# OFA-Sys/ONE-PEACE

Hardware: NVIDIA H100
Metric: encoder_samples_per_sec (higher is better)
Workload: dtype bf16

## Files before the change

one_peace_b200/csrc/common.cuh:

```cuda
#pragma once
#include <cuda.h>
#include <cuda_bf16.h>
#include <cuda_runtime.h>
#include <stdint.h>
#include <stdio.h>
#include <stdlib.h>

#define OPB_DEVICE __device__ __forceinline__

#define OPB_OK 0
#define OPB_ERR_INVALID 1
#define OPB_ERR_CUDA 2
#define OPB_ERR_UNSUPPORTED 3

namespace opb {

OPB_DEVICE uint32_t smem_u32(const void* p) {
  return static_cast<uint32_t>(__cvta_generic_to_shared(p));
}
OPB_DEVICE uint32_t lane_id() { return threadIdx.x & 31; }

OPB_DEVICE bool elect_one() {
  uint32_t pred = 0;
  asm volatile(
      "{\n\t"
      ".reg .pred P;\n\t"
      "elect.sync _|P, 0xffffffff;\n\t"
      "selp.b32 %0, 1, 0, P;\n\t"
      "}\n"
      : "=r"(pred));
  return pred != 0;
}

OPB_DEVICE uint64_t globaltimer_ns() {
  uint64_t t;
  asm volatile("mov.u64 %0, %%globaltimer;" : "=l"(t));
  return t;
}

OPB_DEVICE void mbar_init(uint64_t* bar, uint32_t count) {
  asm volatile("mbarrier.init.shared::cta.b64 [%0], %1;" ::"r"(smem_u32(bar)), "r"(count) : "memory");
}
OPB_DEVICE void fence_barrier_init() { asm volatile("fence.mbarrier_init.release.cluster;" ::: "memory"); }
OPB_DEVICE void fence_proxy_async() { asm volatile("fence.proxy.async.shared::cta;" ::: "memory"); }

OPB_DEVICE void mbar_arrive_expect_tx(uint64_t* bar, uint32_t bytes) {
  asm volatile("mbarrier.arrive.expect_tx.shared::cta.b64 _, [%0], %1;" ::"r"(smem_u32(bar)), "r"(bytes)
               : "memory");
}
OPB_DEVICE void mbar_arrive(uint64_t* bar) {
  asm volatile("mbarrier.arrive.shared::cta.b64 _, [%0];" ::"r"(smem_u32(bar)) : "memory");
}
OPB_DEVICE bool mbar_try_wait(uint64_t* bar, uint32_t parity) {
  uint32_t ok;
  asm volatile(
      "{\n\t"
      ".reg .pred P;\n\t"
      "mbarrier.try_wait.parity.shared::cta.b64 P, [%1], %2;\n\t"
      "selp.b32 %0, 1, 0, P;\n\t"
      "}\n"
      : "=r"(ok)
      : "r"(smem_u32(bar)), "r"(parity)
      : "memory");
  return ok != 0;
}

#ifndef OPB_WATCHDOG_NS
#define OPB_WATCHDOG_NS 4000000000ull
#endif
OPB_DEVICE void mbar_wait(uint64_t* bar, uint32_t parity) {
  if (mbar_try_wait(bar, parity)) return;
  uint64_t t0 = globaltimer_ns();
  uint32_t spins = 0;
  while (!mbar_try_wait(bar, parity)) {
    if ((++spins & 0x3ff) == 0) {
      if (globaltimer_ns() - t0 > OPB_WATCHDOG_NS) {
        printf("[opb] mbarrier watchdog: block %d thread %d bar@%u parity %u\n", (int)blockIdx.x,
               (int)threadIdx.x, smem_u32(bar), parity);
        __trap();
      }
    }
  }
}

OPB_DEVICE void mbar_wait_quiet(uint64_t* bar, uint32_t parity) {
  if (mbar_try_wait(bar, parity)) return;
  const uint64_t t0 = globaltimer_ns();
  while (!mbar_try_wait(bar, parity)) {
    if (globaltimer_ns() - t0 > OPB_WATCHDOG_NS) __trap();
  }
}

OPB_DEVICE uint64_t wgmma_desc_sw128(uint32_t smem_addr, uint32_t lbo) {
  uint64_t d = 0;
  d |= static_cast<uint64_t>((smem_addr & 0x3FFFFu) >> 4);
  d |= static_cast<uint64_t>((lbo >> 4) & 0x3FFFu) << 16;
  d |= static_cast<uint64_t>(1024 >> 4) << 32;
  d |= static_cast<uint64_t>(1) << 62;
  return d;
}

OPB_DEVICE void wgmma_fence() { asm volatile("wgmma.fence.sync.aligned;" ::: "memory"); }
OPB_DEVICE void wgmma_commit() { asm volatile("wgmma.commit_group.sync.aligned;" ::: "memory"); }
template <int N>
OPB_DEVICE void wgmma_wait() { asm volatile("wgmma.wait_group.sync.aligned %0;" ::"n"(N) : "memory"); }

static inline int sm_count() {
  static int n = 0;
  if (n == 0) {
    int dev = 0;
    cudaGetDevice(&dev);
    cudaDeviceGetAttribute(&n, cudaDevAttrMultiProcessorCount, dev);
  }
  return n;
}

OPB_DEVICE void tma_prefetch_desc(const CUtensorMap* m) {
  asm volatile("prefetch.tensormap [%0];" ::"l"(reinterpret_cast<uint64_t>(m)) : "memory");
}

OPB_DEVICE void tma_load_2d(const CUtensorMap* m, uint64_t* bar, void* dst, int32_t c0, int32_t c1) {
  asm volatile(
      "cp.async.bulk.tensor.2d.shared::cluster.global.mbarrier::complete_tx::bytes [%0], [%1, {%3, %4}], [%2];"
      :
      : "r"(smem_u32(dst)), "l"(reinterpret_cast<uint64_t>(m)), "r"(smem_u32(bar)), "r"(c0), "r"(c1)
      : "memory");
}
OPB_DEVICE void tma_load_3d(const CUtensorMap* m, uint64_t* bar, void* dst, int32_t c0, int32_t c1, int32_t c2) {
  asm volatile(
      "cp.async.bulk.tensor.3d.shared::cluster.global.mbarrier::complete_tx::bytes [%0], [%1, {%3, %4, %5}], [%2];"
      :
      : "r"(smem_u32(dst)), "l"(reinterpret_cast<uint64_t>(m)), "r"(smem_u32(bar)), "r"(c0), "r"(c1), "r"(c2)
      : "memory");
}
// ... 63 lines not shown
```

one_peace_b200/csrc/gemm_wgmma.cu:

```cuda
#include "common.cuh"
#include "gemm.h"

#include <mutex>

namespace opb {

constexpr int kBlockM = 128;
constexpr int kBlockN = 256;
constexpr int kBlockK = 64;
constexpr int kStages = 4;
constexpr int kStagesTmaOut = 3;
constexpr int kABytes = kBlockM * kBlockK * 2;
constexpr int kBBytes = kBlockN * kBlockK * 2;
constexpr int kStageBytes = kABytes + kBBytes;
constexpr int kThreads = 384;
constexpr int kBandM = 8;
constexpr int kResidBatch = 16;

struct EpiOperands {
  float2 row[kBlockM];
  float colsum[kBlockN], bias[kBlockN], gamma[kBlockN], colscale[kBlockN];
};
constexpr int kStagerThreads = 96;
constexpr int kOutBoxBytes = 64 * 128;
constexpr int kOutStageBytes = 4 * kOutBoxBytes;
constexpr int smem_bytes(int stages, bool tma_out) {
  return stages * kStageBytes + (tma_out ? 2 * kOutStageBytes : 0) + 1024 + 2 * sizeof(EpiOperands) + 1024;
}
constexpr int kSmemBytes = smem_bytes(kStages, false);
constexpr int kSmemBytesTmaOut = smem_bytes(kStagesTmaOut, true);
static_assert(kSmemBytesTmaOut <= 227 * 1024, "output staging does not fit next to the stage ring");

struct GemmGeom {
  int M, N, K;
  int kb_inner;
  int num_k_blocks;
  int groups;
  int a_group_c0;
  int b_group_rows;
  int a_mn;
  int b_mn;
  int kb_per_piece;
  int m_pad;
  float* split_ws;
};

OPB_DEVICE void fence_acc(float (&d)[128]) {
#pragma unroll
  for (int i = 0; i < 128; ++i) asm volatile("" : "+f"(d[i])::"memory");
}

template <int TA, int TB>
OPB_DEVICE void wgmma_m64n256k16(float (&d)[128], uint64_t desc_a, uint64_t desc_b, uint32_t scale_d) {
  asm volatile(
      "{\n\t"
      ".reg .pred p;\n\t"
      "setp.ne.b32 p, %130, 0;\n\t"
      "wgmma.mma_async.sync.aligned.m64n256k16.f32.bf16.bf16 "
      "{"
      "%0, %1, %2, %3, %4, %5, %6, %7, %8, %9, %10, %11, %12, %13, %14, %15, "
      "%16, %17, %18, %19, %20, %21, %22, %23, %24, %25, %26, %27, %28, %29, %30, %31, "
      "%32, %33, %34, %35, %36, %37, %38, %39, %40, %41, %42, %43, %44, %45, %46, %47, "
      "%48, %49, %50, %51, %52, %53, %54, %55, %56, %57, %58, %59, %60, %61, %62, %63, "
      "%64, %65, %66, %67, %68, %69, %70, %71, %72, %73, %74, %75, %76, %77, %78, %79, "
      "%80, %81, %82, %83, %84, %85, %86, %87, %88, %89, %90, %91, %92, %93, %94, %95, "
      "%96, %97, %98, %99, %100, %101, %102, %103, %104, %105, %106, %107, %108, %109, %110, %111, "
      "%112, %113, %114, %115, %116, %117, %118, %119, %120, %121, %122, %123, %124, %125, %126, %127"
      "}, %128, %129, p, 1, 1, %131, %132;\n\t"
      "}\n"
      : "+f"(d[0]), "+f"(d[1]), "+f"(d[2]), "+f"(d[3]), "+f"(d[4]), "+f"(d[5]), "+f"(d[6]), "+f"(d[7]),
        "+f"(d[8]), "+f"(d[9]), "+f"(d[10]), "+f"(d[11]), "+f"(d[12]), "+f"(d[13]), "+f"(d[14]), "+f"(d[15]),
        "+f"(d[16]), "+f"(d[17]), "+f"(d[18]), "+f"(d[19]), "+f"(d[20]), "+f"(d[21]), "+f"(d[22]), "+f"(d[23]),
        "+f"(d[24]), "+f"(d[25]), "+f"(d[26]), "+f"(d[27]), "+f"(d[28]), "+f"(d[29]), "+f"(d[30]), "+f"(d[31]),
        "+f"(d[32]), "+f"(d[33]), "+f"(d[34]), "+f"(d[35]), "+f"(d[36]), "+f"(d[37]), "+f"(d[38]), "+f"(d[39]),
        "+f"(d[40]), "+f"(d[41]), "+f"(d[42]), "+f"(d[43]), "+f"(d[44]), "+f"(d[45]), "+f"(d[46]), "+f"(d[47]),
        "+f"(d[48]), "+f"(d[49]), "+f"(d[50]), "+f"(d[51]), "+f"(d[52]), "+f"(d[53]), "+f"(d[54]), "+f"(d[55]),
        "+f"(d[56]), "+f"(d[57]), "+f"(d[58]), "+f"(d[59]), "+f"(d[60]), "+f"(d[61]), "+f"(d[62]), "+f"(d[63]),
        "+f"(d[64]), "+f"(d[65]), "+f"(d[66]), "+f"(d[67]), "+f"(d[68]), "+f"(d[69]), "+f"(d[70]), "+f"(d[71]),
        "+f"(d[72]), "+f"(d[73]), "+f"(d[74]), "+f"(d[75]), "+f"(d[76]), "+f"(d[77]), "+f"(d[78]), "+f"(d[79]),
        "+f"(d[80]), "+f"(d[81]), "+f"(d[82]), "+f"(d[83]), "+f"(d[84]), "+f"(d[85]), "+f"(d[86]), "+f"(d[87]),
        "+f"(d[88]), "+f"(d[89]), "+f"(d[90]), "+f"(d[91]), "+f"(d[92]), "+f"(d[93]), "+f"(d[94]), "+f"(d[95]),
        "+f"(d[96]), "+f"(d[97]), "+f"(d[98]), "+f"(d[99]), "+f"(d[100]), "+f"(d[101]), "+f"(d[102]), "+f"(d[103]),
        "+f"(d[104]), "+f"(d[105]), "+f"(d[106]), "+f"(d[107]), "+f"(d[108]), "+f"(d[109]), "+f"(d[110]), "+f"(d[111]),
        "+f"(d[112]), "+f"(d[113]), "+f"(d[114]), "+f"(d[115]), "+f"(d[116]), "+f"(d[117]), "+f"(d[118]), "+f"(d[119]),
        "+f"(d[120]), "+f"(d[121]), "+f"(d[122]), "+f"(d[123]), "+f"(d[124]), "+f"(d[125]), "+f"(d[126]), "+f"(d[127])
      : "l"(desc_a), "l"(desc_b), "r"(scale_d), "n"(TA), "n"(TB));
}

template <bool kFusedVar = false>
OPB_DEVICE void load_ln_stats(const GemmEpilogue& ep, int row, int M, float& mu, float& rs) {
  mu = 0.f; rs = 1.f;
  const int rc = row < M ? row : M - 1;
  if (ep.ln_partial != nullptr) {
    float s1 = 0.f, s2 = 0.f;
#pragma unroll 8
    for (int p = 0; p < ep.ln_parts; ++p) {
      const float2 v = *reinterpret_cast<const float2*>(ep.ln_partial + (static_cast<long>(p) * M + rc) * 2);
      s1 += v.x; s2 += v.y;
    }
    mu = s1 / ep.ln_dim;
    const float ex2 = s2 / ep.ln_dim;
    const float var = kFusedVar ? fmaf(-mu, mu, ex2) : __fsub_rn(ex2, __fmul_rn(mu, mu));
    rs = rsqrtf(fmaxf(var, 0.f) + ep.ln_eps);
  } else if (ep.ln_mu != nullptr) {
    mu = ep.ln_mu[rc];
    rs = ep.ln_rstd[rc];
  }
}

OPB_DEVICE float2 ldf2(const float* p) { return *reinterpret_cast<const float2*>(p); }
OPB_DEVICE float quad_sum(float v) {
  v += __shfl_xor_sync(0xffffffffu, v, 1);
  return v + __shfl_xor_sync(0xffffffffu, v, 2);
}
// ... 208 lines not shown
          st_sq += u0 * u0 + u1 * u1;
          if constexpr (kTmaOut) packed[j] = pack_bf16x2(u0, u1);
          else if (row_ok) *reinterpret_cast<uint32_t*>(out + tc) = pack_bf16x2(u0, u1);
        }
        if constexpr (kTmaOut) stage_out_row(out_stage, h, packed);
        st_sum = quad_sum(st_sum);
        st_sq = quad_sum(st_sq);
        if (row_ok && quad == 0 && ep.stats_out != nullptr) {
          *reinterpret_cast<float2*>(ep.stats_out + (static_cast<long>(n_blk * 2) * M + row) * 2) = make_float2(st_sum, st_sq);
          *reinterpret_cast<float2*>(ep.stats_out + (static_cast<long>(n_blk * 2 + 1) * M + row) * 2) = make_float2(0.f, 0.f);
        }
      } else {
        uint32_t packed[32];
#pragma unroll
        for (int jb = 0; jb < 32; jb += kResidBatch) {
          float2 res[kResidBatch];
          if constexpr (EPI == EPI_RESID_F32) {
            if (ep.resid != nullptr && row_ok) {
              const float* rp = ep.resid + res_row * ep.ldr + gcol0;
#pragma unroll
              for (int jj = 0; jj < kResidBatch; ++jj) {
                const int tc = col0 + 8 * (jb + jj) + 2 * quad;
                if (tc < N) res[jj] = ldf2(rp + tc);
              }
            }
          }
#pragma unroll
          for (int jj = 0; jj < kResidBatch; ++jj) {
            const int j = jb + jj;
            const int lc = 8 * j + 2 * quad;
            const int tc = col0 + lc;
            if (!kTmaOut && tc >= N) continue;
            const int col = gcol0 + tc;
            float x0 = d[4 * j + 2 * h], x1 = d[4 * j + 2 * h + 1];
            if (has_ln) {
              const float2 c = ldf2(st->colsum + lc);
              x0 = rs * (x0 - mu * c.x); x1 = rs * (x1 - mu * c.y);
            }
            if (ep.bias != nullptr) {
              const float2 b = ldf2(st->bias + lc);
              x0 += b.x; x1 += b.y;
            }
            if constexpr (EPI == EPI_STORE_BF16 || EPI == EPI_GELU_BF16) {
              if (ep.colscale != nullptr) {
                const float2 s = ldf2(st->colscale + lc);
                x0 *= s.x; x1 *= s.y;
              }
              if constexpr (EPI == EPI_GELU_BF16) { x0 = gelu_erf(x0); x1 = gelu_erf(x1); }
              if constexpr (kTmaOut) {
                packed[j] = pack_bf16x2(x0, x1);
              } else {
                if (row_ok) *reinterpret_cast<uint32_t*>(reinterpret_cast<__nv_bfloat16*>(ep.out) + out_row * ep.ldo + col) = pack_bf16x2(x0, x1);
              }
            } else {
              if constexpr (EPI == EPI_RESID_F32) {
                if (ep.gamma != nullptr) {
                  const float2 g = ldf2(st->gamma + lc);
                  x0 *= g.x; x1 *= g.y;
                }
                if (ep.resid != nullptr && row_ok) {
                  x0 += res[jj].x; x1 += res[jj].y;
                }
                st_sum += x0 + x1;
                st_sq += x0 * x0 + x1 * x1;
                if (row_ok && ep.out_bf16 != nullptr)
                  *reinterpret_cast<uint32_t*>(reinterpret_cast<__nv_bfloat16*>(ep.out_bf16) + out_row * ep.ldo_bf16 + col) = pack_bf16x2(x0, x1);
              }
              if (row_ok) *reinterpret_cast<float2*>(reinterpret_cast<float*>(ep.out) + out_row * ep.ldo + col) = make_float2(x0, x1);
            }
          }
        }
        if constexpr (kTmaOut) stage_out_row(out_stage, h, packed);
        if constexpr (EPI == EPI_RESID_F32) {
          st_sum = quad_sum(st_sum);
          st_sq = quad_sum(st_sq);
          if (row_ok && quad == 0 && ep.stats_out != nullptr)
            *reinterpret_cast<float2*>(ep.stats_out + (static_cast<long>(n_blk) * M + row) * 2) = make_float2(st_sum, st_sq);
        }
      }
    }
  }
}

struct TileCoord {
  int piece, grp, m_blk, n_blk;
};
OPB_DEVICE TileCoord tile_coord(int unit, int num_m_tiles, int num_n_tiles, int groups) {
  const int per_group = num_m_tiles * num_n_tiles;
  TileCoord c;
  c.piece = unit / (per_group * groups);
  const int tile = unit - c.piece * per_group * groups;
  c.grp = tile / per_group;
  const int tin = tile - c.grp * per_group;
  const int band = tin / (kBandM * num_n_tiles);
  const int m0 = band * kBandM;
  const int band_rows = min(kBandM, num_m_tiles - m0);
  const int r = tin - m0 * num_n_tiles;
  c.m_blk = m0 + r % band_rows;
  c.n_blk = r / band_rows;
  return c;
}

template <int EPI, int S, bool kTmaOut>
OPB_DEVICE void gemm_body(const CUtensorMap& tm_a, const CUtensorMap& tm_b, const CUtensorMap* tm_out, const GemmEpilogue& ep,
                          const GemmGeom& geo) {
  extern __shared__ __align__(1024) uint8_t smem_raw[];
  uint8_t* smem = smem_raw;
  if ((smem_u32(smem) & 1023u) != 0) __trap();
  uint8_t* out_stage = smem + S * kStageBytes;
  uint8_t* bars = out_stage + (kTmaOut ? 2 * kOutStageBytes : 0);
  uint64_t* full = reinterpret_cast<uint64_t*>(bars);
  uint64_t* empty = full + S;
  uint64_t* epi_full = empty + S;
  uint64_t* epi_empty = epi_full + 2;
  EpiOperands* epi_ops = reinterpret_cast<EpiOperands*>(bars + 1024);

  const int wg = threadIdx.x >> 7;
  const int num_m_tiles = (geo.M + kBlockM - 1) / kBlockM;
  const int num_n_tiles = (geo.N + kBlockN - 1) / kBlockN;
  const int pieces = geo.kb_per_piece > 0 ? (geo.num_k_blocks + geo.kb_per_piece - 1) / geo.kb_per_piece : 1;
  const int units = num_m_tiles * num_n_tiles * geo.groups * pieces;
  const bool staged = epi_staged(EPI) && (kTmaOut || geo.kb_per_piece == 0);

  if (threadIdx.x == 0) {
    tma_prefetch_desc(&tm_a);
    tma_prefetch_desc(&tm_b);
    if constexpr (kTmaOut) tma_prefetch_desc(tm_out);
    for (int i = 0; i < S; ++i) {
      mbar_init(&full[i], 1);
      mbar_init(&empty[i], 8);
    }
    for (int i = 0; i < 2; ++i) {
      mbar_init(&epi_full[i], kStagerThreads);
      mbar_init(&epi_empty[i], 8);
    }
    fence_barrier_init();
  }
  __syncthreads();

  if (wg == 0) {
    asm volatile("setmaxnreg.dec.sync.aligned.u32 40;");
    if (threadIdx.x == 0) {
      uint32_t it = 0;
      for (int unit = blockIdx.x; unit < units; unit += gridDim.x) {
        const TileCoord tc = tile_coord(unit, num_m_tiles, num_n_tiles, geo.groups);
        const int kb0 = geo.kb_per_piece > 0 ? tc.piece * geo.kb_per_piece : 0;
        const int kb1 = geo.kb_per_piece > 0 ? min(geo.num_k_blocks, kb0 + geo.kb_per_piece) : geo.num_k_blocks;
        const int a_row = tc.m_blk * kBlockM;
        const int b_row = tc.grp * geo.b_group_rows + tc.n_blk * kBlockN;
        const int a_c0 = tc.grp * geo.a_group_c0;
        int kin = kb0 % geo.kb_inner, tap = kb0 / geo.kb_inner;
        for (int kb = kb0; kb < kb1; ++kb, ++it) {
          const uint32_t s = it % S;
          mbar_wait_quiet(&empty[s], ((it / S) & 1) ^ 1);
          uint8_t* sa = smem + s * kStageBytes;
          uint8_t* sb = sa + kABytes;
          mbar_arrive_expect_tx(&full[s], kStageBytes);
          if (geo.a_mn) {
#pragma unroll
            for (int i = 0; i < kBlockM / 64; ++i) tma_load_2d(&tm_a, &full[s], sa + i * 8192, a_row + 64 * i, kb * kBlockK);
          } else {
            tma_load_3d(&tm_a, &full[s], sa, a_c0 + kin * kBlockK, tap, a_row);
          }
          if (geo.b_mn) {
#pragma unroll
            for (int i = 0; i < kBlockN / 64; ++i) tma_load_2d(&tm_b, &full[s], sb + i * 8192, b_row + 64 * i, kb * kBlockK);
          } else {
            tma_load_2d(&tm_b, &full[s], sb, kb * kBlockK, b_row);
          }
          if (++kin == geo.kb_inner) { kin = 0; ++tap; }
        }
      }
    } else if (threadIdx.x >= 32 && staged) {
      uint32_t j = 0;
      for (int unit = blockIdx.x; unit < units; unit += gridDim.x, ++j) {
        const TileCoord tc = tile_coord(unit, num_m_tiles, num_n_tiles, geo.groups);
        mbar_wait_quiet(&epi_empty[j & 1], ((j >> 1) & 1) ^ 1);
        stage_epi_operands<EPI>(&epi_ops[j & 1], ep, geo, tc.m_blk, tc.n_blk, tc.grp, threadIdx.x - 32);
        mbar_arrive(&epi_full[j & 1]);
      }
    }
  } else {
    asm volatile("setmaxnreg.inc.sync.aligned.u32 232;");
    const int cw = wg - 1;
    uint8_t* my_stage = out_stage + cw * kOutStageBytes;
    float d[128];
#pragma unroll
    for (int i = 0; i < 128; ++i) d[i] = 0.f;
    uint32_t it = 0, j = 0;
    for (int unit = blockIdx.x; unit < units; unit += gridDim.x, ++j) {
      const TileCoord tc = tile_coord(unit, num_m_tiles, num_n_tiles, geo.groups);
      const int kb0 = geo.kb_per_piece > 0 ? tc.piece * geo.kb_per_piece : 0;
      const int kb1 = geo.kb_per_piece > 0 ? min(geo.num_k_blocks, kb0 + geo.kb_per_piece) : geo.num_k_blocks;
      if (geo.a_mn) {
        if (geo.b_mn) mainloop<1, 1, S>(d, smem, full, empty, kb1 - kb0, cw, it);
        else mainloop<1, 0, S>(d, smem, full, empty, kb1 - kb0, cw, it);
      } else {
        if (geo.b_mn) mainloop<0, 1, S>(d, smem, full, empty, kb1 - kb0, cw, it);
        else mainloop<0, 0, S>(d, smem, full, empty, kb1 - kb0, cw, it);
      }
      it += kb1 - kb0;
      if (!kTmaOut && geo.kb_per_piece > 0) {
        const int t = threadIdx.x & 127, lane = t & 31;
        const int r0 = tc.m_blk * kBlockM + cw * 64 + (t >> 5) * 16 + (lane >> 2);
        float* w = geo.split_ws + static_cast<long>(tc.piece) * geo.m_pad * geo.N;
#pragma unroll
        for (int h = 0; h < 2; ++h) {
#pragma unroll
          for (int c = 0; c < 32; ++c) {
            const int col = tc.n_blk * kBlockN + 8 * c + 2 * (lane & 3);
            if (col < geo.N)
              *reinterpret_cast<float2*>(w + static_cast<long>(r0 + 8 * h) * geo.N + col) = make_float2(d[4 * c + 2 * h], d[4 * c + 2 * h + 1]);
          }
        }
      } else if (staged) {
        mbar_wait_quiet(&epi_full[j & 1], (j >> 1) & 1);
        if constexpr (kTmaOut) acquire_out_stage(cw);
        epilogue<EPI, kTmaOut>(d, ep, geo, &epi_ops[j & 1], smem_u32(my_stage), tc.m_blk, tc.n_blk, tc.grp, cw);
        __syncwarp();
        if ((threadIdx.x & 31) == 0) mbar_arrive(&epi_empty[j & 1]);
        if constexpr (kTmaOut) {
          constexpr int cols_per_tile = EPI == EPI_GEGLU_BF16 ? kBlockN / 2 : kBlockN;
          store_out_tile(*tm_out, my_stage, tc.m_blk * kBlockM + cw * 64, tc.n_blk * cols_per_tile, geo.M,
                         EPI == EPI_GEGLU_BF16 ? geo.N / 2 : geo.N, cols_per_tile / 64, cw);
        }
      } else {
        epilogue<EPI, false>(d, ep, geo, nullptr, 0, tc.m_blk, tc.n_blk, tc.grp, cw);
      }
    }
    if constexpr (kTmaOut) {
      if ((threadIdx.x & 127) == 0) bulk_wait_all<0>();
    }
  }
}

template <int EPI>
__global__ void __launch_bounds__(kThreads, 1)
gemm_bf16_kernel(const __grid_constant__ CUtensorMap tm_a, const __grid_constant__ CUtensorMap tm_b, const GemmEpilogue ep,
                 const GemmGeom geo) {
  gemm_body<EPI, kStages, false>(tm_a, tm_b, nullptr, ep, geo);
}

template <int EPI>
__global__ void __launch_bounds__(kThreads, 1)
gemm_bf16_tma_out_kernel(const __grid_constant__ CUtensorMap tm_a, const __grid_constant__ CUtensorMap tm_b,
                         const __grid_constant__ CUtensorMap tm_out, const GemmEpilogue ep, const GemmGeom geo) {
  static_assert(EPI == EPI_STORE_BF16 || EPI == EPI_GELU_BF16 || EPI == EPI_GEGLU_BF16, "bf16 epilogues only");
  gemm_body<EPI, kStagesTmaOut, true>(tm_a, tm_b, &tm_out, ep, geo);
}

__global__ void __launch_bounds__(256)
gemm_split_epilogue_kernel(const GemmEpilogue ep, const GemmGeom geo, int pieces, int epi) {
  __shared__ float red[2][8];
  const int M = geo.M, N = geo.N;
  const int row = blockIdx.x;
  float mu, rs;
  if (ep.ln_partial != nullptr) {
    float s1 = 0.f, s2 = 0.f;
    for (int p = threadIdx.x; p < ep.ln_parts; p += blockDim.x) {
      const float2 v = *reinterpret_cast<const float2*>(ep.ln_partial + (static_cast<long>(p) * M + row) * 2);
      s1 += v.x; s2 += v.y;
    }
    s1 = warp_sum(s1); s2 = warp_sum(s2);
    if ((threadIdx.x & 31) == 0) { red[0][threadIdx.x >> 5] = s1; red[1][threadIdx.x >> 5] = s2; }
    __syncthreads();
    s1 = s2 = 0.f;
    for (int i = 0; i < 8; ++i) { s1 += red[0][i]; s2 += red[1][i]; }
    mu = s1 / ep.ln_dim;
    rs = rsqrtf(fmaxf(s2 / ep.ln_dim - mu * mu, 0.f) + ep.ln_eps);
  } else {
    load_ln_stats(ep, row, M, mu, rs);
  }
  const int t = blockIdx.y;
  const int col = t * kBlockN + threadIdx.x;
  const long slab = static_cast<long>(geo.m_pad) * N;
  float x = 0.f;
  if (col < N) {
    const float* w = geo.split_ws + static_cast<long>(row) * N + col;
    for (int p = 0; p < pieces; ++p) x += w[p * slab];
    if (ep.ln_colsum) x = rs * (x - mu * ep.ln_colsum[col]);
    if (ep.bias) x += ep.bias[col];
    if (epi == EPI_STORE_BF16) {
      if (ep.colscale) x *= ep.colscale[col];
      reinterpret_cast<__nv_bfloat16*>(ep.out)[static_cast<long>(row) * ep.ldo + col] = __float2bfloat16(x);
    } else {
      if (ep.gamma) x *= ep.gamma[col];
      if (ep.resid) x += ep.resid[static_cast<long>(row) * ep.ldr + col];
      reinterpret_cast<float*>(ep.out)[static_cast<long>(row) * ep.ldo + col] = x;
      if (ep.out_bf16) reinterpret_cast<__nv_bfloat16*>(ep.out_bf16)[static_cast<long>(row) * ep.ldo_bf16 + col] = __float2bfloat16(x);
    }
  }
  if (ep.stats_out != nullptr) {
    const float s1 = warp_sum(x), s2 = warp_sum(x * x);
    __syncthreads();
    if ((threadIdx.x & 31) == 0) { red[0][threadIdx.x >> 5] = s1; red[1][threadIdx.x >> 5] = s2; }
    __syncthreads();
    if (threadIdx.x == 0) {
      float a = 0.f, b = 0.f;
      for (int i = 0; i < 8; ++i) { a += red[0][i]; b += red[1][i]; }
      *reinterpret_cast<float2*>(ep.stats_out + (static_cast<long>(t) * M + row) * 2) = make_float2(a, b);
    }
  }
}

typedef CUresult (*PFN_encodeTiled)(CUtensorMap*, CUtensorMapDataType, cuuint32_t, void*, const cuuint64_t*,
                                    const cuuint64_t*, const cuuint32_t*, const cuuint32_t*, CUtensorMapInterleave,
                                    CUtensorMapSwizzle, CUtensorMapL2promotion, CUtensorMapFloatOOBfill);

static PFN_encodeTiled get_encode_fn() {
  static PFN_encodeTiled fn = nullptr;
  static std::once_flag once;
  std::call_once(once, [] {
    void* p = nullptr;
    cudaDriverEntryPointQueryResult qres;
    if (cudaGetDriverEntryPoint("cuTensorMapEncodeTiled", &p, cudaEnableDefault, &qres) == cudaSuccess &&
        qres == cudaDriverEntryPointSuccess) {
      fn = reinterpret_cast<PFN_encodeTiled>(p);
    }
  });
  return fn;
}

int make_tmap_bf16_2d(CUtensorMap* out, const void* ptr, uint64_t rows, uint64_t cols, uint64_t ld,
                      uint32_t box_rows) {
  PFN_encodeTiled enc = get_encode_fn();
  if (enc == nullptr) return OPB_ERR_CUDA;
  if ((reinterpret_cast<uintptr_t>(ptr) & 15) != 0 || (ld * 2) % 16 != 0) return OPB_ERR_INVALID;
  cuuint64_t gdim[2] = {cols, rows};
  cuuint64_t gstride[1] = {ld * 2};
  cuuint32_t box[2] = {static_cast<cuuint32_t>(kBlockK), box_rows};
  cuuint32_t estr[2] = {1, 1};
  CUresult r = enc(out, CU_TENSOR_MAP_DATA_TYPE_BFLOAT16, 2, const_cast<void*>(ptr), gdim, gstride, box, estr,
                   CU_TENSOR_MAP_INTERLEAVE_NONE, CU_TENSOR_MAP_SWIZZLE_128B, CU_TENSOR_MAP_L2_PROMOTION_L2_256B,
                   CU_TENSOR_MAP_FLOAT_OOB_FILL_NONE);
  return r == CUDA_SUCCESS ? OPB_OK : OPB_ERR_CUDA;
}

int make_tmap_bf16_3d(CUtensorMap* out, const void* ptr, uint64_t k_inner, uint64_t taps, uint64_t tap_stride,
                      uint64_t rows, uint64_t row_stride, uint32_t box_rows) {
  PFN_encodeTiled enc = get_encode_fn();
  if (enc == nullptr) return OPB_ERR_CUDA;
  if ((reinterpret_cast<uintptr_t>(ptr) & 15) != 0 || (tap_stride * 2) % 16 != 0 || (row_stride * 2) % 16 != 0)
    return OPB_ERR_INVALID;
  cuuint64_t gdim[3] = {k_inner, taps, rows};
  cuuint64_t gstride[2] = {tap_stride * 2, row_stride * 2};
  cuuint32_t box[3] = {static_cast<cuuint32_t>(kBlockK), 1, box_rows};
  cuuint32_t estr[3] = {1, 1, 1};
  CUresult r = enc(out, CU_TENSOR_MAP_DATA_TYPE_BFLOAT16, 3, const_cast<void*>(ptr), gdim, gstride, box, estr,
                   CU_TENSOR_MAP_INTERLEAVE_NONE, CU_TENSOR_MAP_SWIZZLE_128B, CU_TENSOR_MAP_L2_PROMOTION_L2_256B,
                   CU_TENSOR_MAP_FLOAT_OOB_FILL_NONE);
  return r == CUDA_SUCCESS ? OPB_OK : OPB_ERR_CUDA;
}

int make_tmap_bf16_batched(CUtensorMap* out, const void* ptr, uint64_t cols, uint64_t rows, uint64_t ld, uint64_t batches,
                           uint64_t batch_stride, uint32_t box_rows) {
  PFN_encodeTiled enc = get_encode_fn();
  if (enc == nullptr) return OPB_ERR_CUDA;
  if ((reinterpret_cast<uintptr_t>(ptr) & 15) != 0 || (ld * 2) % 16 != 0 || (batch_stride * 2) % 16 != 0)
    return OPB_ERR_INVALID;
  cuuint64_t gdim[3] = {cols, rows, batches};
  cuuint64_t gstride[2] = {ld * 2, batch_stride * 2};
  cuuint32_t box[3] = {static_cast<cuuint32_t>(kBlockK), box_rows, 1};
  cuuint32_t estr[3] = {1, 1, 1};
  CUresult r = enc(out, CU_TENSOR_MAP_DATA_TYPE_BFLOAT16, 3, const_cast<void*>(ptr), gdim, gstride, box, estr,
                   CU_TENSOR_MAP_INTERLEAVE_NONE, CU_TENSOR_MAP_SWIZZLE_128B, CU_TENSOR_MAP_L2_PROMOTION_L2_256B,
                   CU_TENSOR_MAP_FLOAT_OOB_FILL_NONE);
  return r == CUDA_SUCCESS ? OPB_OK : OPB_ERR_CUDA;
}

template <int EPI, bool kTmaOut>
static int launch_gemm(const CUtensorMap& ta, const CUtensorMap& tb, const CUtensorMap* to, const GemmEpilogue& ep,
                       const GemmGeom& geo, cudaStream_t stream) {
  constexpr int smem = kTmaOut ? kSmemBytesTmaOut : kSmemBytes;
  const void* kern;
  if constexpr (kTmaOut) kern = reinterpret_cast<const void*>(gemm_bf16_tma_out_kernel<EPI>);
  else kern = reinterpret_cast<const void*>(gemm_bf16_kernel<EPI>);
  static int resident = 0;
  if (resident == 0) {
    if (cudaFuncSetAttribute(kern, cudaFuncAttributeMaxDynamicSharedMemorySize, smem) != cudaSuccess)
      return OPB_ERR_CUDA;
    int per_sm = 0;
    if (cudaOccupancyMaxActiveBlocksPerMultiprocessor(&per_sm, kern, kThreads, smem) != cudaSuccess || per_sm < 1)
      return OPB_ERR_CUDA;
    resident = per_sm * sm_count();
  }
  const int pieces = geo.kb_per_piece > 0 ? (geo.num_k_blocks + geo.kb_per_piece - 1) / geo.kb_per_piece : 1;
  const long units = static_cast<long>((geo.M + kBlockM - 1) / kBlockM) * ((geo.N + kBlockN - 1) / kBlockN) * geo.groups * pieces;
  const unsigned grid = static_cast<unsigned>(units < resident ? units : resident);
  if constexpr (kTmaOut) gemm_bf16_tma_out_kernel<EPI><<<grid, kThreads, smem, stream>>>(ta, tb, *to, ep, geo);
  else gemm_bf16_kernel<EPI><<<grid, kThreads, smem, stream>>>(ta, tb, ep, geo);
  return cudaGetLastError() == cudaSuccess ? OPB_OK : OPB_ERR_CUDA;
}

static int dispatch_gemm(int epi, const CUtensorMap& ta, const CUtensorMap& tb, const CUtensorMap* to, const GemmEpilogue& ep,
                         const GemmGeom& geo, cudaStream_t stream) {
  if (to != nullptr) {
    switch (epi) {
      case EPI_STORE_BF16: return launch_gemm<EPI_STORE_BF16, true>(ta, tb, to, ep, geo, stream);
      case EPI_GELU_BF16: return launch_gemm<EPI_GELU_BF16, true>(ta, tb, to, ep, geo, stream);
      case EPI_GEGLU_BF16: return launch_gemm<EPI_GEGLU_BF16, true>(ta, tb, to, ep, geo, stream);
      default: return OPB_ERR_INVALID;
    }
  }
  switch (epi) {
    case EPI_STORE_BF16: return launch_gemm<EPI_STORE_BF16, false>(ta, tb, nullptr, ep, geo, stream);
    case EPI_GELU_BF16: return launch_gemm<EPI_GELU_BF16, false>(ta, tb, nullptr, ep, geo, stream);
    case EPI_GEGLU_BF16: return launch_gemm<EPI_GEGLU_BF16, false>(ta, tb, nullptr, ep, geo, stream);
    case EPI_RESID_F32: return launch_gemm<EPI_RESID_F32, false>(ta, tb, nullptr, ep, geo, stream);
    case EPI_STORE_F32: return launch_gemm<EPI_STORE_F32, false>(ta, tb, nullptr, ep, geo, stream);
    case EPI_LSE_PARTIAL: return launch_gemm<EPI_LSE_PARTIAL, false>(ta, tb, nullptr, ep, geo, stream);
    case EPI_SOFTMAX_GRAD: return launch_gemm<EPI_SOFTMAX_GRAD, false>(ta, tb, nullptr, ep, geo, stream);
    default: return OPB_ERR_INVALID;
  }
}

static bool tma_out_applies(int epi, const GemmEpilogue& ep, const GemmGeom& geo, long out_cols) {
  return (epi == EPI_STORE_BF16 || epi == EPI_GELU_BF16 || epi == EPI_GEGLU_BF16) && geo.kb_per_piece == 0 && geo.groups == 1 &&
         ep.out_group == 0 && (reinterpret_cast<uintptr_t>(ep.out) & 15) == 0 && (ep.ldo * 2) % 16 == 0 && ep.ldo >= out_cols;
}

struct ByteSpan {
  const char* begin;
  const char* end;
};
static ByteSpan row_span(const void* p, long lo, long hi, long ld, long cols, int esz) {
  const char* c = static_cast<const char*>(p);
  return {c + lo * ld * esz, c + (hi * ld + cols) * esz};
}
static bool spans_meet(const ByteSpan& a, const ByteSpan& b) { return a.begin < b.end && b.begin < a.end; }

static bool resid_aliasing_ok(const GemmEpilogue& ep, int M, long cols) {
  if (ep.resid == nullptr) return true;
  auto out_row = [&](long m) {
    return ep.out_group > 0 ? (m / ep.out_group) * ep.out_group_stride + m % ep.out_group + ep.out_row_offset : m;
  };
  const long g = ep.out_group > 0 ? ep.out_group : M, last = M - 1, q = last / g;
  const long corners[5] = {0, (g < M ? g : M) - 1, q * g, last, q > 0 ? q * g - 1 : 0};
  long lo = out_row(0), hi = lo;
  for (long m : corners) {
    lo = out_row(m) < lo ? out_row(m) : lo;
    hi = out_row(m) > hi ? out_row(m) : hi;
  }
  long rlo = lo, rhi = hi;
  if (ep.resid_period > 0) {
    rlo = ep.resid_row_offset;
    rhi = rlo + (ep.resid_period < M ? ep.resid_period : M) - 1;
  }
  const ByteSpan res = row_span(ep.resid, rlo, rhi, ep.ldr, cols, 4);
  if (ep.out_bf16 != nullptr && spans_meet(res, row_span(ep.out_bf16, lo, hi, ep.ldo_bf16, cols, 2))) return false;
  if (!spans_meet(res, row_span(ep.out, lo, hi, ep.ldo, cols, 4))) return true;
  return ep.resid == ep.out && ep.ldr == ep.ldo && ep.resid_period == 0;
}

static GemmGeom plain_geom(int M, int N, int K) {
  GemmGeom geo;
  geo.M = M; geo.N = N; geo.K = K;
  geo.num_k_blocks = (K + kBlockK - 1) / kBlockK;
  geo.kb_inner = geo.num_k_blocks;
  geo.groups = 1;
  geo.a_group_c0 = 0;
  geo.b_group_rows = 0;
  geo.a_mn = geo.b_mn = 0;
  geo.kb_per_piece = 0;
  geo.m_pad = 0;
  geo.split_ws = nullptr;
  return geo;
}

int gemm_bf16(const void* A, int lda, const void* B, int ldb, int M, int N, int K, int epi, const GemmEpilogue& ep,
              int cta_group, cudaStream_t stream) {
  if (M <= 0 || N <= 0 || K <= 0) return OPB_ERR_INVALID;
  if (K % 8 != 0 || N % 8 != 0 || lda % 8 != 0 || ldb % 8 != 0) return OPB_ERR_INVALID;
  if (epi == EPI_GEGLU_BF16 && N % kBlockN != 0) return OPB_ERR_INVALID;
  if (cta_group < 0 || cta_group > 2) return OPB_ERR_INVALID;
  if (epi == EPI_RESID_F32 && !resid_aliasing_ok(ep, M, N)) return OPB_ERR_INVALID;
  GemmGeom geo = plain_geom(M, N, K);
  const int m_tiles = (M + kBlockM - 1) / kBlockM, n_tiles = (N + kBlockN - 1) / kBlockN;
  const bool split_ok = (epi == EPI_RESID_F32 || (epi == EPI_STORE_BF16 && ep.stats_out == nullptr)) && ep.workspace != nullptr &&
                        ep.out_group == 0 && ep.resid_period == 0 && M <= 2 * kBlockM && geo.num_k_blocks >= 8;
  int pieces = 1;
  if (split_ok) {
    const long slab_bytes = static_cast<long>(m_tiles) * kBlockM * N * 4;
    pieces = sm_count() / (m_tiles * n_tiles);
    if (pieces > geo.num_k_blocks / 2) pieces = geo.num_k_blocks / 2;
    if (pieces > ep.workspace_bytes / slab_bytes) pieces = static_cast<int>(ep.workspace_bytes / slab_bytes);
    if (pieces >= 2) {
      geo.kb_per_piece = (geo.num_k_blocks + pieces - 1) / pieces;
      pieces = (geo.num_k_blocks + geo.kb_per_piece - 1) / geo.kb_per_piece;
      geo.m_pad = m_tiles * kBlockM;
      geo.split_ws = reinterpret_cast<float*>(ep.workspace);
    }
  }
  CUtensorMap ta, tb;
  int rc = make_tmap_bf16_3d(&ta, A, K, 1, lda, M, lda, kBlockM);
  if (rc != OPB_OK) return rc;
  rc = make_tmap_bf16_2d(&tb, B, N, K, ldb, kBlockN);
  if (rc != OPB_OK) return rc;
  const long out_cols = epi == EPI_GEGLU_BF16 ? N / 2 : N;
  CUtensorMap to;
  const bool tma_out = tma_out_applies(epi, ep, geo, out_cols);
  if (tma_out && (rc = make_tmap_bf16_2d(&to, ep.out, M, out_cols, ep.ldo, 64)) != OPB_OK) return rc;
  rc = dispatch_gemm(epi, ta, tb, tma_out ? &to : nullptr, ep, geo, stream);
  if (rc != OPB_OK || geo.kb_per_piece == 0) return rc;
  gemm_split_epilogue_kernel<<<dim3(M, n_tiles), 256, 0, stream>>>(ep, geo, pieces, epi);
  return cudaGetLastError() == cudaSuccess ? OPB_OK : OPB_ERR_CUDA;
}

int gemm_bf16_t(const void* A, int lda, int a_mn, const void* B, int ldb, int b_mn, int M, int N, int K, int epi,
                const GemmEpilogue& ep, int cta_group, cudaStream_t stream) {
  if (M <= 0 || N <= 0 || K <= 0 || lda % 8 != 0 || ldb % 8 != 0 || N % 8 != 0) return OPB_ERR_INVALID;
  if (epi != EPI_STORE_BF16 && epi != EPI_STORE_F32) return OPB_ERR_INVALID;
  if ((!a_mn && K % 8 != 0) || (!b_mn && K % 8 != 0) || (a_mn && M % 8 != 0)) return OPB_ERR_INVALID;
  if (cta_group < 0 || cta_group > 2) return OPB_ERR_INVALID;
  GemmGeom geo = plain_geom(M, N, K);
  geo.a_mn = a_mn ? 1 : 0;
  geo.b_mn = b_mn ? 1 : 0;
  CUtensorMap ta, tb;
  int rc = a_mn ? make_tmap_bf16_2d(&ta, A, K, M, lda, 64) : make_tmap_bf16_3d(&ta, A, K, 1, lda, M, lda, kBlockM);
  if (rc != OPB_OK) return rc;
  rc = b_mn ? make_tmap_bf16_2d(&tb, B, K, N, ldb, 64) : make_tmap_bf16_2d(&tb, B, N, K, ldb, kBlockN);
  if (rc != OPB_OK) return rc;
  CUtensorMap to;
  const bool tma_out = tma_out_applies(epi, ep, geo, N);
  if (tma_out && (rc = make_tmap_bf16_2d(&to, ep.out, M, N, ep.ldo, 64)) != OPB_OK) return rc;
  return dispatch_gemm(epi, ta, tb, tma_out ? &to : nullptr, ep, geo, stream);
}

int gemm_bf16_grouped_window(const void* X, const void* W, int rows, int groups, int c_pad, int taps, int n_per_group,
                             int epi, const GemmEpilogue& ep, cudaStream_t stream) {
  if (rows <= 0 || groups <= 0 || taps <= 0 || n_per_group <= 0) return OPB_ERR_INVALID;
  if (c_pad % kBlockK != 0 || n_per_group % 8 != 0 || n_per_group > kBlockN) return OPB_ERR_INVALID;
  if (epi == EPI_GEGLU_BF16 || epi == EPI_LSE_PARTIAL || epi == EPI_SOFTMAX_GRAD) return OPB_ERR_INVALID;
  if (epi == EPI_RESID_F32 && !resid_aliasing_ok(ep, rows, static_cast<long>(groups) * n_per_group)) return OPB_ERR_INVALID;
  GemmGeom geo = plain_geom(rows, n_per_group, taps * c_pad);
  geo.kb_inner = c_pad / kBlockK;
  geo.num_k_blocks = taps * geo.kb_inner;
  geo.groups = groups;
  geo.a_group_c0 = c_pad;
  geo.b_group_rows = n_per_group;
  const long row_stride = static_cast<long>(groups) * c_pad;
  CUtensorMap ta, tb;
  int rc = make_tmap_bf16_3d(&ta, X, row_stride, taps, row_stride, rows, row_stride, kBlockM);
  if (rc != OPB_OK) return rc;
  rc = make_tmap_bf16_2d(&tb, W, static_cast<uint64_t>(groups) * n_per_group, geo.K, geo.K, kBlockN);
  if (rc != OPB_OK) return rc;
  return dispatch_gemm(epi, ta, tb, nullptr, ep, geo, stream);
}

}
```

Measured before the change: 793.6.

## Stream residual epilogue through the TMA stage ring with bulk loads and stores

Adds a residual-add GEMM path in which the producer warp TMA-loads fp32 residual tiles into the mainloop stage ring after each tile's K loop. The epilogue warpgroups then combine them in shared memory and TMA-store fp32 and optional bf16 outputs chunk by chunk, releasing stages as the stores finish reading. This replaces per-thread scattered global residual reads and output writes with bulk asynchronous transfers. The cost is extra producer/consumer handshakes that serialize the epilogue with the next tile's loads, plus stricter alignment requirements.

```diff
diff --git a/one_peace_b200/csrc/common.cuh b/one_peace_b200/csrc/common.cuh
--- a/one_peace_b200/csrc/common.cuh
+++ b/one_peace_b200/csrc/common.cuh
@@ -50,6 +50,9 @@
 }
 OPB_DEVICE void mbar_arrive(uint64_t* bar) {
   asm volatile("mbarrier.arrive.shared::cta.b64 _, [%0];" ::"r"(smem_u32(bar)) : "memory");
+}
+OPB_DEVICE void mbar_arrive_count(uint64_t* bar, uint32_t count) {
+  asm volatile("mbarrier.arrive.shared::cta.b64 _, [%0], %1;" ::"r"(smem_u32(bar)), "r"(count) : "memory");
 }
 OPB_DEVICE bool mbar_try_wait(uint64_t* bar, uint32_t parity) {
   uint32_t ok;
diff --git a/one_peace_b200/csrc/gemm_wgmma.cu b/one_peace_b200/csrc/gemm_wgmma.cu
--- a/one_peace_b200/csrc/gemm_wgmma.cu
+++ b/one_peace_b200/csrc/gemm_wgmma.cu
@@ -30,6 +30,10 @@
 constexpr int kSmemBytes = smem_bytes(kStages, false);
 constexpr int kSmemBytesTmaOut = smem_bytes(kStagesTmaOut, true);
 static_assert(kSmemBytesTmaOut <= 227 * 1024, "output staging does not fit next to the stage ring");
+constexpr int kChunks = kBlockN / 64;
+constexpr int kResidBoxBytes = kBlockM * 128;
+constexpr int kChunkBf16Offset = 2 * kResidBoxBytes;
+static_assert(kChunkBf16Offset + kBlockM * 128 == kStageBytes, "a residual chunk fills one stage");
 
 struct GemmGeom {
   int M, N, K;
@@ -404,6 +408,89 @@
   }
 }
 
+template <int S>
+OPB_DEVICE void epilogue_resid_ring(const float (&d)[128], const GemmEpilogue& ep, const GemmGeom& geo, const EpiOperands* st,
+                                    uint8_t* smem, uint64_t* full, uint64_t* empty, const CUtensorMap& tm_out,
+                                    const CUtensorMap& tm_out_bf16, uint32_t it, int m_blk, int n_blk, int cw) {
+  const int M = geo.M, N = geo.N;
+  const int t = threadIdx.x & 127;
+  const int lane = t & 31;
+  const int quad = lane & 3;
+  const int rloc = cw * 64 + (t >> 5) * 16 + (lane >> 2);
+  const int rbase = m_blk * kBlockM + rloc;
+  const int row0 = m_blk * kBlockM + cw * 64;
+  const bool has_ln = ep.ln_colsum != nullptr;
+  const bool has_rows = ep.ln_partial != nullptr || ep.ln_mu != nullptr;
+  float st_sum[2] = {0.f, 0.f}, st_sq[2] = {0.f, 0.f};
+#pragma unroll
+  for (int c = 0; c < kChunks; ++c) {
+    const uint32_t s = (it + c) % S;
+    mbar_wait_quiet(&full[s], ((it + c) / S) & 1);
+    uint8_t* stage = smem + s * kStageBytes;
+#pragma unroll
+    for (int h = 0; h < 2; ++h) {
+      const int r = rloc + 8 * h;
+      const bool row_ok = rbase + 8 * h < M;
+      const float2 mr = has_rows ? st->row[r] : make_float2(0.f, 1.f);
+      const float mu = mr.x, rs = mr.y;
+#pragma unroll
+      for (int jj = 0; jj < 8; ++jj) {
+        const int j = 8 * c + jj;
+        const int lc = 8 * j + 2 * quad;
+        float2* f = reinterpret_cast<float2*>(stage + (jj >> 2) * kResidBoxBytes + sw128_off(r, 2 * (jj & 3) + (quad >> 1)) +
+                                              8 * (quad & 1));
+        float x0 = d[4 * j + 2 * h], x1 = d[4 * j + 2 * h + 1];
+        if (has_ln) {
+          const float2 cs = ldf2(st->colsum + lc);
+          x0 = rs * (x0 - mu * cs.x); x1 = rs * (x1 - mu * cs.y);
+        }
+        if (ep.bias != nullptr) {
+          const float2 b = ldf2(st->bias + lc);
+          x0 += b.x; x1 += b.y;
+        }
+        if (ep.gamma != nullptr) {
+          const float2 g = ldf2(st->gamma + lc);
+          x0 *= g.x; x1 *= g.y;
+        }
+        if (row_ok) {
+          const float2 res = *f;
+          x0 += res.x; x1 += res.y;
+        }
+        st_sum[h] += x0 + x1;
+        st_sq[h] += x0 * x0 + x1 * x1;
+        *f = make_float2(x0, x1);
+        *reinterpret_cast<uint32_t*>(stage + kChunkBf16Offset + sw128_off(r, jj) + 4 * quad) = pack_bf16x2(x0, x1);
+      }
+    }
+    fence_proxy_async();
+    warpgroup_bar_sync(cw);
+    if (t == 0) {
+      const int col = n_blk * kBlockN + 64 * c;
+      if (row0 < M) {
+        for (int b = 0; b < 2; ++b)
+          if (col + 32 * b < N) tma_store_2d(&tm_out, stage + b * kResidBoxBytes + cw * 64 * 128, col + 32 * b, row0);
+        if (ep.out_bf16 != nullptr && col < N) tma_store_2d(&tm_out_bf16, stage + kChunkBf16Offset + cw * 64 * 128, col, row0);
+      }
+      bulk_commit();
+      if (c > 0) {
+        bulk_wait_read<1>();
+        mbar_arrive_count(&empty[(it + c - 1) % S], 4);
+      }
+      if (c == kChunks - 1) {
+        bulk_wait_read<0>();
+        mbar_arrive_count(&empty[s], 4);
+      }
+    }
+  }
+#pragma unroll
+  for (int h = 0; h < 2; ++h) {
+    const int row = rbase + 8 * h;
+    const float s1 = quad_sum(st_sum[h]), s2 = quad_sum(st_sq[h]);
+    if (row < M && quad == 0 && ep.stats_out != nullptr)
+      *reinterpret_cast<float2*>(ep.stats_out + (static_cast<long>(n_blk) * M + row) * 2) = make_float2(s1, s2);
+  }
+}
+
 struct TileCoord {
   int piece, grp, m_blk, n_blk;
 };
@@ -423,9 +510,13 @@
   return c;
 }
 
-template <int EPI, int S, bool kTmaOut>
-OPB_DEVICE void gemm_body(const CUtensorMap& tm_a, const CUtensorMap& tm_b, const CUtensorMap* tm_out, const GemmEpilogue& ep,
-                          const GemmGeom& geo) {
+enum class OutPath { kDirect, kTmaBf16, kResidRing };
+
+template <int EPI, int S, OutPath kPath>
+OPB_DEVICE void gemm_body(const CUtensorMap& tm_a, const CUtensorMap& tm_b, const CUtensorMap* tm_out, const CUtensorMap* tm_res,
+                          const CUtensorMap* tm_out_bf16, const GemmEpilogue& ep, const GemmGeom& geo) {
+  constexpr bool kTmaOut = kPath == OutPath::kTmaBf16;
+  constexpr bool kRing = kPath == OutPath::kResidRing;
   extern __shared__ __align__(1024) uint8_t smem_raw[];
   uint8_t* smem = smem_raw;
   if ((smem_u32(smem) & 1023u) != 0) __trap();
@@ -442,12 +533,16 @@
   const int num_n_tiles = (geo.N + kBlockN - 1) / kBlockN;
   const int pieces = geo.kb_per_piece > 0 ? (geo.num_k_blocks + geo.kb_per_piece - 1) / geo.kb_per_piece : 1;
   const int units = num_m_tiles * num_n_tiles * geo.groups * pieces;
-  const bool staged = epi_staged(EPI) && (kTmaOut || geo.kb_per_piece == 0);
+  const bool staged = epi_staged(EPI) && (kTmaOut || kRing || geo.kb_per_piece == 0);
 
   if (threadIdx.x == 0) {
     tma_prefetch_desc(&tm_a);
     tma_prefetch_desc(&tm_b);
-    if constexpr (kTmaOut) tma_prefetch_desc(tm_out);
+    if constexpr (kTmaOut || kRing) tma_prefetch_desc(tm_out);
+    if constexpr (kRing) {
+      tma_prefetch_desc(tm_res);
+      if (ep.out_bf16 != nullptr) tma_prefetch_desc(tm_out_bf16);
+    }
     for (int i = 0; i < S; ++i) {
       mbar_init(&full[i], 1);
       mbar_init(&empty[i], 8);
@@ -492,6 +587,16 @@
           }
           if (++kin == geo.kb_inner) { kin = 0; ++tap; }
         }
+        if constexpr (kRing) {
+          for (int c = 0; c < kChunks; ++c, ++it) {
+            const uint32_t s = it % S;
+            mbar_wait_quiet(&empty[s], ((it / S) & 1) ^ 1);
+            uint8_t* sr = smem + s * kStageBytes;
+            mbar_arrive_expect_tx(&full[s], 2 * kResidBoxBytes);
+            for (int b = 0; b < 2; ++b)
+              tma_load_2d(tm_res, &full[s], sr + b * kResidBoxBytes, tc.n_blk * kBlockN + 64 * c + 32 * b, a_row);
+          }
+        }
       }
     } else if (threadIdx.x >= 32 && staged) {
       uint32_t j = 0;
@@ -522,7 +627,7 @@
         else mainloop<0, 0, S>(d, smem, full, empty, kb1 - kb0, cw, it);
       }
       it += kb1 - kb0;
-      if (!kTmaOut && geo.kb_per_piece > 0) {
+      if (kPath == OutPath::kDirect && geo.kb_per_piece > 0) {
         const int t = threadIdx.x & 127, lane = t & 31;
         const int r0 = tc.m_blk * kBlockM + cw * 64 + (t >> 5) * 16 + (lane >> 2);
         float* w = geo.split_ws + static_cast<long>(tc.piece) * geo.m_pad * geo.N;
@@ -538,7 +643,12 @@
       } else if (staged) {
         mbar_wait_quiet(&epi_full[j & 1], (j >> 1) & 1);
         if constexpr (kTmaOut) acquire_out_stage(cw);
-        epilogue<EPI, kTmaOut>(d, ep, geo, &epi_ops[j & 1], smem_u32(my_stage), tc.m_blk, tc.n_blk, tc.grp, cw);
+        if constexpr (kRing) {
+          epilogue_resid_ring<S>(d, ep, geo, &epi_ops[j & 1], smem, full, empty, *tm_out, *tm_out_bf16, it, tc.m_blk, tc.n_blk, cw);
+          it += kChunks;
+        } else {
+          epilogue<EPI, kTmaOut>(d, ep, geo, &epi_ops[j & 1], smem_u32(my_stage), tc.m_blk, tc.n_blk, tc.grp, cw);
+        }
         __syncwarp();
         if ((threadIdx.x & 31) == 0) mbar_arrive(&epi_empty[j & 1]);
         if constexpr (kTmaOut) {
@@ -550,7 +660,7 @@
         epilogue<EPI, false>(d, ep, geo, nullptr, 0, tc.m_blk, tc.n_blk, tc.grp, cw);
       }
     }
-    if constexpr (kTmaOut) {
+    if constexpr (kTmaOut || kRing) {
       if ((threadIdx.x & 127) == 0) bulk_wait_all<0>();
     }
   }
@@ -560,7 +670,7 @@
 __global__ void __launch_bounds__(kThreads, 1)
 gemm_bf16_kernel(const __grid_constant__ CUtensorMap tm_a, const __grid_constant__ CUtensorMap tm_b, const GemmEpilogue ep,
                  const GemmGeom geo) {
-  gemm_body<EPI, kStages, false>(tm_a, tm_b, nullptr, ep, geo);
+  gemm_body<EPI, kStages, OutPath::kDirect>(tm_a, tm_b, nullptr, nullptr, nullptr, ep, geo);
 }
 
 template <int EPI>
@@ -568,7 +678,16 @@
 gemm_bf16_tma_out_kernel(const __grid_constant__ CUtensorMap tm_a, const __grid_constant__ CUtensorMap tm_b,
                          const __grid_constant__ CUtensorMap tm_out, const GemmEpilogue ep, const GemmGeom geo) {
   static_assert(EPI == EPI_STORE_BF16 || EPI == EPI_GELU_BF16 || EPI == EPI_GEGLU_BF16, "bf16 epilogues only");
-  gemm_body<EPI, kStagesTmaOut, true>(tm_a, tm_b, &tm_out, ep, geo);
+  gemm_body<EPI, kStagesTmaOut, OutPath::kTmaBf16>(tm_a, tm_b, &tm_out, nullptr, nullptr, ep, geo);
+}
+
+template <int EPI>
+__global__ void __launch_bounds__(kThreads, 1)
+gemm_bf16_resid_tma_kernel(const __grid_constant__ CUtensorMap tm_a, const __grid_constant__ CUtensorMap tm_b,
+                           const __grid_constant__ CUtensorMap tm_res, const __grid_constant__ CUtensorMap tm_out,
+                           const __grid_constant__ CUtensorMap tm_out_bf16, const GemmEpilogue ep, const GemmGeom geo) {
+  static_assert(EPI == EPI_RESID_F32, "the residual epilogue only");
+  gemm_body<EPI, kStages, OutPath::kResidRing>(tm_a, tm_b, &tm_out, &tm_res, &tm_out_bf16, ep, geo);
 }
 
 __global__ void __launch_bounds__(256)
@@ -658,6 +777,20 @@
   return r == CUDA_SUCCESS ? OPB_OK : OPB_ERR_CUDA;
 }
 
+static int make_tmap_f32_2d(CUtensorMap* out, const void* ptr, uint64_t rows, uint64_t cols, uint64_t ld, uint32_t box_rows) {
+  PFN_encodeTiled enc = get_encode_fn();
+  if (enc == nullptr) return OPB_ERR_CUDA;
+  if ((reinterpret_cast<uintptr_t>(ptr) & 15) != 0 || (ld * 4) % 16 != 0) return OPB_ERR_INVALID;
+  cuuint64_t gdim[2] = {cols, rows};
+  cuuint64_t gstride[1] = {ld * 4};
+  cuuint32_t box[2] = {32, box_rows};
+  cuuint32_t estr[2] = {1, 1};
+  CUresult r = enc(out, CU_TENSOR_MAP_DATA_TYPE_FLOAT32, 2, const_cast<void*>(ptr), gdim, gstride, box, estr,
+                   CU_TENSOR_MAP_INTERLEAVE_NONE, CU_TENSOR_MAP_SWIZZLE_128B, CU_TENSOR_MAP_L2_PROMOTION_L2_256B,
+                   CU_TENSOR_MAP_FLOAT_OOB_FILL_NONE);
+  return r == CUDA_SUCCESS ? OPB_OK : OPB_ERR_CUDA;
+}
+
 int make_tmap_bf16_3d(CUtensorMap* out, const void* ptr, uint64_t k_inner, uint64_t taps, uint64_t tap_stride,
                       uint64_t rows, uint64_t row_stride, uint32_t box_rows) {
   PFN_encodeTiled enc = get_encode_fn();
@@ -690,12 +823,14 @@
   return r == CUDA_SUCCESS ? OPB_OK : OPB_ERR_CUDA;
 }
 
-template <int EPI, bool kTmaOut>
+template <int EPI, OutPath kPath>
 static int launch_gemm(const CUtensorMap& ta, const CUtensorMap& tb, const CUtensorMap* to, const GemmEpilogue& ep,
                        const GemmGeom& geo, cudaStream_t stream) {
+  constexpr bool kTmaOut = kPath == OutPath::kTmaBf16;
   constexpr int smem = kTmaOut ? kSmemBytesTmaOut : kSmemBytes;
   const void* kern;
   if constexpr (kTmaOut) kern = reinterpret_cast<const void*>(gemm_bf16_tma_out_kernel<EPI>);
+  else if constexpr (kPath == OutPath::kResidRing) kern = reinterpret_cast<const void*>(gemm_bf16_resid_tma_kernel<EPI>);
   else kern = reinterpret_cast<const void*>(gemm_bf16_kernel<EPI>);
   static int resident = 0;
   if (resident == 0) {
@@ -709,29 +844,33 @@
   const int pieces = geo.kb_per_piece > 0 ? (geo.num_k_blocks + geo.kb_per_piece - 1) / geo.kb_per_piece : 1;
   const long units = static_cast<long>((geo.M + kBlockM - 1) / kBlockM) * ((geo.N + kBlockN - 1) / kBlockN) * geo.groups * pieces;
   const unsigned grid = static_cast<unsigned>(units < resident ? units : resident);
-  if constexpr (kTmaOut) gemm_bf16_tma_out_kernel<EPI><<<grid, kThreads, smem, stream>>>(ta, tb, *to, ep, geo);
+  if constexpr (kTmaOut) gemm_bf16_tma_out_kernel<EPI><<<grid, kThreads, smem, stream>>>(ta, tb, to[0], ep, geo);
+  else if constexpr (kPath == OutPath::kResidRing)
+    gemm_bf16_resid_tma_kernel<EPI><<<grid, kThreads, smem, stream>>>(ta, tb, to[0], to[1], to[2], ep, geo);
   else gemm_bf16_kernel<EPI><<<grid, kThreads, smem, stream>>>(ta, tb, ep, geo);
   return cudaGetLastError() == cudaSuccess ? OPB_OK : OPB_ERR_CUDA;
 }
 
 static int dispatch_gemm(int epi, const CUtensorMap& ta, const CUtensorMap& tb, const CUtensorMap* to, const GemmEpilogue& ep,
                          const GemmGeom& geo, cudaStream_t stream) {
+  constexpr OutPath D = OutPath::kDirect, T = OutPath::kTmaBf16;
   if (to != nullptr) {
     switch (epi) {
-      case EPI_STORE_BF16: return launch_gemm<EPI_STORE_BF16, true>(ta, tb, to, ep, geo, stream);
-      case EPI_GELU_BF16: return launch_gemm<EPI_GELU_BF16, true>(ta, tb, to, ep, geo, stream);
-      case EPI_GEGLU_BF16: return launch_gemm<EPI_GEGLU_BF16, true>(ta, tb, to, ep, geo, stream);
+      case EPI_STORE_BF16: return launch_gemm<EPI_STORE_BF16, T>(ta, tb, to, ep, geo, stream);
+      case EPI_GELU_BF16: return launch_gemm<EPI_GELU_BF16, T>(ta, tb, to, ep, geo, stream);
+      case EPI_GEGLU_BF16: return launch_gemm<EPI_GEGLU_BF16, T>(ta, tb, to, ep, geo, stream);
+      case EPI_RESID_F32: return launch_gemm<EPI_RESID_F32, OutPath::kResidRing>(ta, tb, to, ep, geo, stream);
       default: return OPB_ERR_INVALID;
     }
   }
   switch (epi) {
-    case EPI_STORE_BF16: return launch_gemm<EPI_STORE_BF16, false>(ta, tb, nullptr, ep, geo, stream);
-    case EPI_GELU_BF16: return launch_gemm<EPI_GELU_BF16, false>(ta, tb, nullptr, ep, geo, stream);
-    case EPI_GEGLU_BF16: return launch_gemm<EPI_GEGLU_BF16, false>(ta, tb, nullptr, ep, geo, stream);
-    case EPI_RESID_F32: return launch_gemm<EPI_RESID_F32, false>(ta, tb, nullptr, ep, geo, stream);
-    case EPI_STORE_F32: return launch_gemm<EPI_STORE_F32, false>(ta, tb, nullptr, ep, geo, stream);
-    case EPI_LSE_PARTIAL: return launch_gemm<EPI_LSE_PARTIAL, false>(ta, tb, nullptr, ep, geo, stream);
-    case EPI_SOFTMAX_GRAD: return launch_gemm<EPI_SOFTMAX_GRAD, false>(ta, tb, nullptr, ep, geo, stream);
+    case EPI_STORE_BF16: return launch_gemm<EPI_STORE_BF16, D>(ta, tb, nullptr, ep, geo, stream);
+    case EPI_GELU_BF16: return launch_gemm<EPI_GELU_BF16, D>(ta, tb, nullptr, ep, geo, stream);
+    case EPI_GEGLU_BF16: return launch_gemm<EPI_GEGLU_BF16, D>(ta, tb, nullptr, ep, geo, stream);
+    case EPI_RESID_F32: return launch_gemm<EPI_RESID_F32, D>(ta, tb, nullptr, ep, geo, stream);
+    case EPI_STORE_F32: return launch_gemm<EPI_STORE_F32, D>(ta, tb, nullptr, ep, geo, stream);
+    case EPI_LSE_PARTIAL: return launch_gemm<EPI_LSE_PARTIAL, D>(ta, tb, nullptr, ep, geo, stream);
+    case EPI_SOFTMAX_GRAD: return launch_gemm<EPI_SOFTMAX_GRAD, D>(ta, tb, nullptr, ep, geo, stream);
     default: return OPB_ERR_INVALID;
   }
 }
@@ -739,6 +878,15 @@
 static bool tma_out_applies(int epi, const GemmEpilogue& ep, const GemmGeom& geo, long out_cols) {
   return (epi == EPI_STORE_BF16 || epi == EPI_GELU_BF16 || epi == EPI_GEGLU_BF16) && geo.kb_per_piece == 0 && geo.groups == 1 &&
          ep.out_group == 0 && (reinterpret_cast<uintptr_t>(ep.out) & 15) == 0 && (ep.ldo * 2) % 16 == 0 && ep.ldo >= out_cols;
+}
+
+static bool resid_ring_applies(int epi, const GemmEpilogue& ep, const GemmGeom& geo) {
+  auto plain = [&](const void* p, long ld, int esz) {
+    return (reinterpret_cast<uintptr_t>(p) & 15) == 0 && (ld * esz) % 16 == 0 && ld >= geo.N;
+  };
+  return epi == EPI_RESID_F32 && geo.kb_per_piece == 0 && geo.groups == 1 && ep.out_group == 0 && ep.resid_period == 0 &&
+         ep.resid != nullptr && plain(ep.resid, ep.ldr, 4) && plain(ep.out, ep.ldo, 4) &&
+         (ep.out_bf16 == nullptr || plain(ep.out_bf16, ep.ldo_bf16, 2));
 }
 
 struct ByteSpan {
@@ -819,10 +967,17 @@
   rc = make_tmap_bf16_2d(&tb, B, N, K, ldb, kBlockN);
   if (rc != OPB_OK) return rc;
   const long out_cols = epi == EPI_GEGLU_BF16 ? N / 2 : N;
-  CUtensorMap to;
+  CUtensorMap to[3];
   const bool tma_out = tma_out_applies(epi, ep, geo, out_cols);
-  if (tma_out && (rc = make_tmap_bf16_2d(&to, ep.out, M, out_cols, ep.ldo, 64)) != OPB_OK) return rc;
-  rc = dispatch_gemm(epi, ta, tb, tma_out ? &to : nullptr, ep, geo, stream);
+  const bool ring = resid_ring_applies(epi, ep, geo);
+  if (tma_out && (rc = make_tmap_bf16_2d(&to[0], ep.out, M, out_cols, ep.ldo, 64)) != OPB_OK) return rc;
+  if (ring) {
+    if ((rc = make_tmap_f32_2d(&to[0], ep.resid, M, N, ep.ldr, kBlockM)) != OPB_OK) return rc;
+    if ((rc = make_tmap_f32_2d(&to[1], ep.out, M, N, ep.ldo, 64)) != OPB_OK) return rc;
+    to[2] = to[1];
+    if (ep.out_bf16 != nullptr && (rc = make_tmap_bf16_2d(&to[2], ep.out_bf16, M, N, ep.ldo_bf16, 64)) != OPB_OK) return rc;
+  }
+  rc = dispatch_gemm(epi, ta, tb, tma_out || ring ? to : nullptr, ep, geo, stream);
   if (rc != OPB_OK || geo.kb_per_piece == 0) return rc;
   gemm_split_epilogue_kernel<<<dim3(M, n_tiles), 256, 0, stream>>>(ep, geo, pieces, epi);
   return cudaGetLastError() == cudaSuccess ? OPB_OK : OPB_ERR_CUDA;
```

New measurement: 827.9, median of 6. +4.3%, better.
